# KiloHertzian/Open-Headstage

Hardware: AMD Instinct MI355X
Metric: Msamples/s stereo 48 kHz (4×512-tap HRIR conv + 10-band EQ); % HBM3E peak (higher is better)
Workload: dtype f32

## Files before the change

open_headstage_amd/csrc/eq_kernels.hip:

```cpp
#include "../../include/ohs_hip.h"
#include "kernels.h"
#include "eq_ring2_body.hpp"
#include "eq_ring64_body.hpp"
#include "eq_quad_ring_body.hpp"
#include "tuning.h"
#ifdef OHS_EXPERIMENTS
#include "experiments/eq_ring_v1.hpp"
#endif

#include <atomic>
#include <cstdlib>

namespace ohs {


template <int SHR, bool GATED>
__device__ __forceinline__ void eq_chunk(long long t0, long long n, int j,
                                         float b0, float b1, float b2, float a1, float a2,
                                         float &s1, float &s2, float &prev, float &c)
{
#pragma unroll
    for (int k = 0; k < 16; ++k) {
        float yv = prev;
        if constexpr (SHR != 0) yv = dpp_mov<0x110 + SHR>(prev, prev);
        const float x = dpp_mov<kRowShr1>(c, prev);
        c = dpp_mov<kRowShl1>(yv, c);
        const float out = s1 + b0 * x;
        const float n1 = (s2 + b1 * x) - a1 * out;
        const float n2 = b2 * x - a2 * out;
        if constexpr (GATED) {
            const long long u = t0 + k - j;
            const bool upd = u >= 0 && u < n;
            s1 = upd ? n1 : s1;
            s2 = upd ? n2 : s2;
            prev = upd ? out : x;
        } else {
            s1 = n1; s2 = n2; prev = out;
        }
    }
}

#include "eq_group_asm.inc"
#define EQ_CLOBBERS "v100", "v102", "v104", "v106", "v108", "v109", "v110", "v111", "v112", "v113", "v114", "memory"
template <int SHR>
__device__ __forceinline__ void eq_group_fast(float b0, v2f b12, v2f a12, float &s1, float &s2, float &o, float &c,
                                              float *sp, const float *lp, const float (&x)[8], float (&nx)[8])
{
#define EQ_GROUP_OUTS [s1] "+v"(s1), [s2] "+v"(s2), [o] "+v"(o), [c] "+v"(c), [n0] "=&v"(nx[0]), [n1] "=&v"(nx[1]), \
                      [n2] "=&v"(nx[2]), [n3] "=&v"(nx[3]), [n4] "=&v"(nx[4]), [n5] "=&v"(nx[5]), [n6] "=&v"(nx[6]),   \
                      [n7] "=&v"(nx[7])
#define EQ_GROUP_INS [b0] "v"(b0), [b12] "v"(b12), [a12] "v"(a12), [sp] "v"(sp), [lp] "v"(lp), [x0] "v"(x[0]),          \
                     [x1] "v"(x[1]), [x2] "v"(x[2]), [x3] "v"(x[3]), [x4] "v"(x[4]), [x5] "v"(x[5]), [x6] "v"(x[6]),   \
                     [x7] "v"(x[7])
    if constexpr (SHR != 0) {
        asm volatile(EQ_GROUP_BODY_SHR : EQ_GROUP_OUTS : EQ_GROUP_INS, [shr] "n"(SHR) : EQ_CLOBBERS);
    } else {
        asm volatile(EQ_GROUP_BODY_NOSHR : EQ_GROUP_OUTS : EQ_GROUP_INS : EQ_CLOBBERS);
    }
#undef EQ_GROUP_OUTS
#undef EQ_GROUP_INS
}


template <int SHR>
__global__ __launch_bounds__(64) void k_eq_pass(const float *in, float *out,
                                                long long stream_stride, long long ch_stride,
                                                long long n, int n_chains, const EqPassTable tab,
                                                float *__restrict__ state, int fp_mode)
{
    ohs_set_fp_mode(fp_mode);
    constexpr int NB = 16 - SHR;
    constexpr int G = 8;
    const int lane = threadIdx.x;
    const int j = lane & 15;
    const long long chain = (long long)blockIdx.x * 4 + (lane >> 4);
    const bool live = chain < n_chains;
    const long long wave_base = (long long)blockIdx.x * 4;
    const long long live_rows = n_chains - wave_base < 4 ? n_chains - wave_base : 4;
    const long long cc = live ? chain : wave_base + (lane >> 4) % live_rows;
    const float *src = in + (cc >> 1) * stream_stride + (cc & 1) * ch_stride;
    float *dst = out + (cc >> 1) * stream_stride + (cc & 1) * ch_stride;

    const float b0 = tab.b0[j], b1 = tab.b1[j], b2 = tab.b2[j], a1 = tab.a1[j], a2 = tab.a2[j];
    const int slot = tab.slot[j];
    float s1 = state[(cc * kEqStateSlots + slot) * 2 + 0];
    float s2 = state[(cc * kEqStateSlots + slot) * 2 + 1];
    float prev = 0.0f, c = 0.0f;

    const long long n_chunks = (n - 1 + NB) / 16 + 1;
    const long long n_groups = (n_chunks + G - 1) / G;
    const long long g_fast_end = n / (16 * G) - 1;

    float cur[G], nxt[G];
#pragma unroll
    for (int e = 0; e < G; ++e) {
        const long long xi = (long long)e * 16 + j;
        cur[e] = (xi < n) ? src[xi] : 0.0f;
    }
    long long g = 0;
    while (g < n_groups) {
        if (g >= 1 && g < g_fast_end) {
            for (; g < g_fast_end; ++g) {
                const float *lp = src + (g + 1) * (16 * G) + j;
                float *sp = dst + g * (16 * G) - 16 - NB + j;
                float xs[8];
#pragma unroll
                for (int e = 0; e < G; ++e) { xs[e] = cur[e]; asm volatile("" : "+v"(xs[e])); }
                eq_group_fast<SHR>(b0, (v2f){b1, b2}, (v2f){a1, a2}, s1, s2, prev, c, sp, lp, xs, nxt);
                eq_wait_loads<8>(nxt);
#pragma unroll
                for (int e = 0; e < G; ++e) cur[e] = nxt[e];
            }
            asm volatile("s_waitcnt vmcnt(0)" ::: "memory");
            continue;
        }
#pragma unroll
        for (int e = 0; e < G; ++e) {
            const long long xi = ((g + 1) * G + e) * 16 + j;
            nxt[e] = (xi < n) ? src[xi] : 0.0f;
        }
#pragma unroll
        for (int e = 0; e < G; ++e) {
            const long long q = g * G + e;
            if (q < n_chunks) {
                const long long t0 = q * 16;
                const long long yi = t0 - 16 - NB + j;
                if (yi >= 0 && yi < n) dst[yi] = c;
                c = cur[e];
                if (t0 >= 16 && t0 + 16 <= n)
                    eq_chunk<SHR, false>(t0, n, j, b0, b1, b2, a1, a2, s1, s2, prev, c);
                else
                    eq_chunk<SHR, true>(t0, n, j, b0, b1, b2, a1, a2, s1, s2, prev, c);
            }
        }
#pragma unroll
        for (int e = 0; e < G; ++e) cur[e] = nxt[e];
        ++g;
    }
    {
        const long long yi = n_chunks * 16 - 16 - NB + j;
        if (yi >= 0 && yi < n) dst[yi] = c;
    }
    if (live && j < NB) {
        state[(cc * kEqStateSlots + slot) * 2 + 0] = s1;
        state[(cc * kEqStateSlots + slot) * 2 + 1] = s2;
    }
}

#ifdef OHS_EXPERIMENTS
#include "experiments/eq_ring_v1_kernel.inc"
#endif

#if defined(OHS_EXPERIMENTS) && defined(OHS_EQ_STAMPS)
#include "experiments/eq_stamps.inc"
#else
#define OHS_EQ_STAMP_BEGIN()
#define OHS_EQ_STAMP_END(wave_id)
#endif
__device__ __forceinline__ bool eq_ring_enter(int xcd_lo, int xcd_n, int prio, int fp_mode, long long &wave_id)
{
    unsigned bid = blockIdx.x;
    if (xcd_n != 8) {
        const unsigned x = (bid & 7u) - (unsigned)xcd_lo;
        if (x >= (unsigned)xcd_n) return false;
        bid = (bid >> 3) * (unsigned)xcd_n + x;
    }
    ohs_set_fp_mode(fp_mode);
    if (prio) __builtin_amdgcn_s_setprio(3);
    wave_id = __builtin_amdgcn_readfirstlane((int)(bid * (blockDim.x >> 6) + (threadIdx.x >> 6)));
    return true;
}

__global__ __launch_bounds__(1024) __attribute__((amdgpu_num_vgpr(16))) void k_eq_ring(const float *in, float *out, long long stream_stride,
                                                 long long ch_stride, long long n, int n_chains, int nb,
                                                 const EqPassTable tab, float *__restrict__ state, int prio, int fp_mode,
                                                 int xcd_lo, int xcd_n, unsigned long long *stamps, int wave_ring)
{
    unsigned bid = blockIdx.x;
    if (xcd_n != 8) {
        const unsigned x = (bid & 7u) - (unsigned)xcd_lo;
        if (x >= (unsigned)xcd_n) return;
        bid = (bid >> 3) * (unsigned)xcd_n + x;
    }
    ohs_set_fp_mode(fp_mode);
    if (prio) __builtin_amdgcn_s_setprio(3);
    const long long wave_id = __builtin_amdgcn_readfirstlane((int)(bid * (blockDim.x >> 6) + (threadIdx.x >> 6)));
    OHS_EQ_STAMP_BEGIN();
    const bool stamp = stamps != nullptr && wave_id == 0;
    unsigned long long srt0 = 0, sck0 = 0;
    if (stamp) { srt0 = __builtin_amdgcn_s_memrealtime(); sck0 = __builtin_amdgcn_s_memtime(); }
    const int ring_form = __builtin_amdgcn_readfirstlane(wave_ring);
#ifdef OHS_EXPERIMENTS
    if (ring_form == 3) eq_quad_ring_wave<kQuadLoopFill>(in, out, stream_stride, ch_stride, n, n_chains, nb, tab, state, wave_id);
    else if (ring_form == 4) eq_quad_ring_wave<kQuadLoopLone>(in, out, stream_stride, ch_stride, n, n_chains, nb, tab, state, wave_id);
    else if (ring_form == 5) eq_quad_ring_wave<kQuadLoopCluster>(in, out, stream_stride, ch_stride, n, n_chains, nb, tab, state, wave_id);
    else
#endif
    if (ring_form == 2) eq_quad_ring_wave(in, out, stream_stride, ch_stride, n, n_chains, nb, tab, state, wave_id);
    else if (ring_form) eq_ring64_wave(in, out, stream_stride, ch_stride, n, n_chains, nb, tab, state, wave_id);
    else eq_ring2_wave(in, out, stream_stride, ch_stride, n, n_chains, nb, tab, state, wave_id);
    if (stamp) {
        const unsigned long long srt1 = __builtin_amdgcn_s_memrealtime(), sck1 = __builtin_amdgcn_s_memtime();
        if ((threadIdx.x & 63) == 0) { stamps[0] = srt0; stamps[1] = srt1; stamps[2] = sck0; stamps[3] = sck1; }
    }
    OHS_EQ_STAMP_END(wave_id);
}

__global__ __launch_bounds__(1024) __attribute__((amdgpu_num_vgpr(16))) void k_eq_ring_streams(const float *in, float *out, long long stream_stride,
                                                 long long ch_stride, long long n, int n_chains,
                                                 const EqStreamTable *__restrict__ stabs, float *__restrict__ state, int prio,
                                                 int fp_mode, int xcd_lo, int xcd_n, int wave_ring)
{
    long long wave_id;
    if (!eq_ring_enter(xcd_lo, xcd_n, prio, fp_mode, wave_id)) return;
    EqPassTable unused;
    if (__builtin_amdgcn_readfirstlane(wave_ring)) eq_ring64_wave_t<true>(in, out, stream_stride, ch_stride, n, n_chains, 0, unused, stabs, state, wave_id);
    else eq_ring2_wave_t<true>(in, out, stream_stride, ch_stride, n, n_chains, 0, unused, stabs, state, wave_id);
}

__global__ __launch_bounds__(1024) void k_eq_ring_sched(const float *in, float *out, long long stream_stride, long long ch_stride,
                                                        long long n, int n_chains, int nb, const EqPassTable tab,
                                                        float *__restrict__ state, int prio, int fp_mode, int xcd_lo, int xcd_n,
                                                        unsigned long long *stamps, const EqRingSched sch)
{
    unsigned bid = blockIdx.x;
    if (xcd_n != 8) {
        const unsigned x = (bid & 7u) - (unsigned)xcd_lo;
        if (x >= (unsigned)xcd_n) return;
        bid = (bid >> 3) * (unsigned)xcd_n + x;
    }
    ohs_set_fp_mode(fp_mode);
    if (prio) __builtin_amdgcn_s_setprio(3);
    const long long wave_id = __builtin_amdgcn_readfirstlane((int)(bid * (blockDim.x >> 6) + (threadIdx.x >> 6)));
    const bool stamp = stamps != nullptr && wave_id == 0;
    unsigned long long srt0 = 0, sck0 = 0;
    if (stamp) { srt0 = __builtin_amdgcn_s_memrealtime(); sck0 = __builtin_amdgcn_s_memtime(); }
    eq_ring64_wave_t<false, true>(in, out, stream_stride, ch_stride, n, n_chains, nb, tab, nullptr, state, wave_id, &sch);
    if (stamp) {
        const unsigned long long srt1 = __builtin_amdgcn_s_memrealtime(), sck1 = __builtin_amdgcn_s_memtime();
        if ((threadIdx.x & 63) == 0) { stamps[0] = srt0; stamps[1] = srt1; stamps[2] = sck0; stamps[3] = sck1; }
    }
}

static int eq_device_cus()
{
    static std::atomic<int> cus_cached{0};
    int cus = cus_cached.load(std::memory_order_relaxed);
    if (cus == 0) {
        int dev = 0;
        if (hipGetDevice(&dev) != hipSuccess ||
            hipDeviceGetAttribute(&cus, hipDeviceAttributeMultiprocessorCount, dev) != hipSuccess || cus <= 0)
            cus = 256;
        cus_cached.store(cus, std::memory_order_relaxed);
    }
    return cus;
}

static EqPlan eq_plan_for(bool one_table, long long stream_stride, long long ch_stride, long long n, int n_chains, int n_bands,
                          bool exact_specials, int xcd_lo, int xcd_n)
{
    return eq_plan(one_table, eq_ring2_addressable(stream_stride, ch_stride, n), n, n_chains, n_bands, exact_specials, xcd_lo, xcd_n,
                   eq_device_cus(), tuning());
}

bool eq_pass_takes_wave_ring(long long stream_stride, long long ch_stride, long long n, int n_chains, int n_bands, bool exact_specials)
{
    return eq_plan_for(true, stream_stride, ch_stride, n, n_chains, n_bands, exact_specials, 0, 8).form == OHS_EQ_FORM_WAVE_RING;
}

template <typename... P, typename... A>
static hipError_t eq_dispatch(void (*kernel)(P...), const EqPlan &p, hipStream_t st, hipEvent_t ev_start, hipEvent_t ev_stop, A... args)
{
    if (!p.valid) return hipErrorInvalidValue;
    const bool launch = p.form != OHS_EQ_FORM_NONE;
    const dim3 grid(p.grid), block(64 * p.wg_waves);
    if (launch && p.form != OHS_EQ_FORM_CONVEYOR && !p.ring_v1 && (ev_start || ev_stop)) {
        hipExtLaunchKernelGGL(kernel, grid, block, p.lds, st, ev_start, ev_stop, 0, static_cast<P>(args)...);
        return hipGetLastError();
    }
    if (ev_start) { hipError_t e = hipEventRecord(ev_start, st); if (e != hipSuccess) return e; }
    if (launch) {
        hipLaunchKernelGGL(kernel, grid, block, p.lds, st, static_cast<P>(args)...);
        hipError_t e = hipGetLastError();
        if (e != hipSuccess) return e;
    }
    return ev_stop ? hipEventRecord(ev_stop, st) : hipSuccess;
}

static bool eq_sched_in_bounds(const EqRingSched &sch, long long n)
{
    return sch.lane_tabs && sch.seg_tab && (n & 511) == 0 && sch.seg_len >= 512 && (sch.seg_len & 511) == 0 && (sch.off0 & 511) == 0 &&
           sch.off0 >= 0 && sch.off0 < sch.seg_len && sch.seg0 >= 0 && sch.seg0 < sch.n_segs;
}

hipError_t launch_eq_ring_sched(const float *in, float *out, long long stream_stride, long long ch_stride, long long n, int n_chains,
                                const EqPassTable &tab, int n_bands, float *state, const EqRingSched &sch, hipStream_t st,
                                int fp_mode, int xcd_lo, int xcd_n, hipEvent_t ev_start, hipEvent_t ev_stop, unsigned long long *stamps)
{
    const EqPlan p = eq_plan_for(true, stream_stride, ch_stride, n, n_chains, n_bands, false, xcd_lo, xcd_n);
    if (p.form != OHS_EQ_FORM_WAVE_RING || !eq_sched_in_bounds(sch, n)) return hipErrorInvalidValue;
    return eq_dispatch(k_eq_ring_sched, p, st, ev_start, ev_stop, in, out, stream_stride, ch_stride, n, n_chains, n_bands, tab, state,
                       p.prio, fp_mode, xcd_lo, xcd_n, stamps, sch);
}

__global__ __launch_bounds__(1024) void k_eq_ring_sched_streams(const float *in, float *out, long long stream_stride,
                                                                long long ch_stride, long long n, int n_chains,
                                                                const EqStreamTable *__restrict__ stabs, float *__restrict__ state,
                                                                int prio, int fp_mode, int xcd_lo, int xcd_n, const EqRingSched sch,
                                                                long long idx_stride)
{
    long long wave_id;
    if (!eq_ring_enter(xcd_lo, xcd_n, prio, fp_mode, wave_id)) return;
    EqPassTable unused;
    eq_ring64_wave_t<true, true>(in, out, stream_stride, ch_stride, n, n_chains, 0, unused, stabs, state, wave_id, &sch, idx_stride);
}

hipError_t launch_eq_ring_sched_streams(const float *in, float *out, long long stream_stride, long long ch_stride, long long n,
                                        int n_chains, const EqStreamTable *d_tabs, float *state, const EqRingSched &sch,
                                        long long idx_stride, hipStream_t st, int fp_mode, int xcd_lo, int xcd_n,
                                        hipEvent_t ev_start, hipEvent_t ev_stop)
{
    const EqPlan p = eq_plan_for(true, stream_stride, ch_stride, n, n_chains, 1, false, xcd_lo, xcd_n);
    if (p.form != OHS_EQ_FORM_WAVE_RING || !d_tabs || !eq_sched_in_bounds(sch, n) || (idx_stride != 0 && idx_stride < sch.n_segs))
        return hipErrorInvalidValue;
    return eq_dispatch(k_eq_ring_sched_streams, p, st, ev_start, ev_stop, in, out, stream_stride, ch_stride, n, n_chains, d_tabs, state,
                       p.prio, fp_mode, xcd_lo, xcd_n, sch, idx_stride);
}

__global__ __launch_bounds__(256) void k_eq_gather_tables(unsigned *__restrict__ dst, const unsigned *__restrict__ tabs,
                                                          const unsigned *__restrict__ idx, long long idx_stride, int n_streams,
                                                          int n_tables, int passes)
{
    constexpr int W = (int)(sizeof(EqStreamTable) / 4);
    const long long i = (long long)blockIdx.x * blockDim.x + threadIdx.x;
    if (i >= (long long)passes * n_streams * W) return;
    const int w = (int)(i % W);
    const long long ps = i / W;
    const int s = (int)(ps % n_streams), pk = (int)(ps / n_streams);
    const unsigned t = idx[(long long)s * idx_stride];
    if (t >= (unsigned)n_tables) return;
    dst[i] = tabs[((long long)pk * n_tables + t) * W + w];
}
hipError_t launch_eq_gather_tables(EqStreamTable *dst, const EqStreamTable *tabs, const unsigned *idx, long long idx_stride,
                                   int n_streams, int n_tables, int passes, hipStream_t st)
{
    static_assert(sizeof(EqStreamTable) % 4 == 0, "EqStreamTable is copied word by word");
    if (!dst || !tabs || !idx || idx_stride < 0 || n_streams <= 0 || n_tables <= 0 || passes <= 0) return hipErrorInvalidValue;
    const long long words = (long long)passes * n_streams * (long long)(sizeof(EqStreamTable) / 4);
    hipLaunchKernelGGL(k_eq_gather_tables, dim3((unsigned)((words + 255) / 256)), dim3(256), 0, st, reinterpret_cast<unsigned *>(dst),
                       reinterpret_cast<const unsigned *>(tabs), idx, idx_stride, n_streams, n_tables, passes);
    return hipGetLastError();
}

bool eq_ring_addressable(long long stream_stride, long long ch_stride, long long n)
{
    return eq_ring2_addressable(stream_stride, ch_stride, n);
}

hipError_t launch_eq_ring_streams(const float *in, float *out, long long stream_stride, long long ch_stride, long long n,
                                  int n_chains, const EqStreamTable *d_tabs, float *state, hipStream_t st, int fp_mode,
                                  int xcd_lo, int xcd_n, hipEvent_t ev_start, hipEvent_t ev_stop, int *form)
{
    EqPlan p = eq_plan_for(false, stream_stride, ch_stride, n, n_chains, 0, false, xcd_lo, xcd_n);
    if (p.form != OHS_EQ_FORM_NONE && !d_tabs) p = EqPlan();
    if (form) *form = p.form;
    return eq_dispatch(k_eq_ring_streams, p, st, ev_start, ev_stop, in, out, stream_stride, ch_stride, n, n_chains, d_tabs, state,
                       p.prio, fp_mode, xcd_lo, xcd_n, p.body);
}

hipError_t launch_eq_pass(const float *in, float *out, long long stream_stride, long long ch_stride,
                          long long n, int n_chains, const EqPassTable &tab, int n_bands, float *state,
                          hipStream_t st, bool exact_specials, int fp_mode, int xcd_lo, int xcd_n,
                          hipEvent_t ev_start, hipEvent_t ev_stop, unsigned long long *stamps, int *form)
{
    const EqPlan p = eq_plan_for(true, stream_stride, ch_stride, n, n_chains, n_bands, exact_specials, xcd_lo, xcd_n);
    if (form) *form = p.form;
    if (p.form == OHS_EQ_FORM_CONVEYOR) {
#define OHS_EQ_CASE(NBV)                                                                                              \
    case NBV:                                                                                                         \
        return eq_dispatch(k_eq_pass<16 - NBV>, p, st, ev_start, ev_stop, in, out, stream_stride, ch_stride, n, n_chains, tab, state, \
                           fp_mode);
        switch (n_bands) {
            OHS_EQ_CASE(1) OHS_EQ_CASE(2) OHS_EQ_CASE(3) OHS_EQ_CASE(4) OHS_EQ_CASE(5) OHS_EQ_CASE(6)
            OHS_EQ_CASE(7) OHS_EQ_CASE(8) OHS_EQ_CASE(9) OHS_EQ_CASE(10) OHS_EQ_CASE(11) OHS_EQ_CASE(12)
            OHS_EQ_CASE(13) OHS_EQ_CASE(14) OHS_EQ_CASE(15) OHS_EQ_CASE(16)
        }
#undef OHS_EQ_CASE
        return hipErrorInvalidValue;
    }
#ifdef OHS_EXPERIMENTS
    if (p.ring_v1)
        return eq_dispatch(k_eq_ring_v1, p, st, ev_start, ev_stop, in, out, stream_stride, ch_stride, n, n_chains, n_bands, tab, state,
                           fp_mode);
#endif
    return eq_dispatch(k_eq_ring, p, st, ev_start, ev_stop, in, out, stream_stride, ch_stride, n, n_chains, n_bands, tab, state, p.prio,
                       fp_mode, xcd_lo, xcd_n, stamps, p.body);
}

__global__ void k_eq_freq_response(const float *__restrict__ coeffs, const int *__restrict__ en, int nb,
                                   float fs, const float *__restrict__ freqs, int n, float *__restrict__ out)
{
    const int i = blockIdx.x * blockDim.x + threadIdx.x;
    if (i >= n) return;
    const float pi = 3.14159265358979323846264338327950288f;
    float rr = 1.0f, ri = 0.0f;
    for (int b = 0; b < nb; ++b) {
        if (!en[b]) continue;
        const float b0 = coeffs[5 * b], b1 = coeffs[5 * b + 1], b2 = coeffs[5 * b + 2];
        const float a1 = coeffs[5 * b + 3], a2 = coeffs[5 * b + 4];
        const float omega = 2.0f * pi * freqs[i] / fs;
        const float zr = 1.0f * cosf(-omega), zi = 1.0f * sinf(-omega);
        const float ns = zr * zr + zi * zi;
        const float ir = zr / ns, ii = -zi / ns;
        const float i2r = ir * ir - ii * ii, i2i = ir * ii + ii * ir;
        const float nr = (b0 + b1 * ir) + b2 * i2r, ni = b1 * ii + b2 * i2i;
        const float dr = (1.0f + a1 * ir) + a2 * i2r, di = a1 * ii + a2 * i2i;
        const float dn = dr * dr + di * di;
        const float qr = (nr * dr + ni * di) / dn, qi = (ni * dr - nr * di) / dn;
        const float tr = rr * qr - ri * qi, ti = rr * qi + ri * qr;
        rr = tr; ri = ti;
    }
    out[i] = hypotf(rr, ri);
}

hipError_t launch_eq_freq_response(const float *d_coeffs, const int *d_en, int nb, float fs,
                                   const float *d_freqs, int n, float *d_out, hipStream_t st)
{
    if (n <= 0) return hipSuccess;
    hipLaunchKernelGGL(k_eq_freq_response, dim3((n + 63) / 64), dim3(64), 0, st, d_coeffs, d_en, nb, fs,
                       d_freqs, n, d_out);
    return hipGetLastError();
}

}
```

open_headstage_amd/csrc/eq_plan.h:

```cpp
#pragma once

#include "../../include/ohs_hip.h"
#include "tuning.h"

namespace ohs {

inline unsigned xcd_grid(unsigned workgroups, int xcd_n)
{
    return xcd_n == 8 ? workgroups : ((workgroups + (unsigned)xcd_n - 1) / (unsigned)xcd_n) * 8u;
}

struct EqPlan {
    bool valid = false;
    int form = OHS_EQ_FORM_NONE;
    int body = 0;
    bool ring_v1 = false;
    int wg_waves = 1;
    unsigned grid = 0;
    int prio = 0;
    int lds = 0;
};

inline EqPlan eq_plan(bool one_table, bool addressable, long long n, int n_chains, int n_bands, bool exact_specials, int xcd_lo,
                      int xcd_n, int cus, const Tuning &tn)
{
    EqPlan p;
    if (n <= 0 || n_chains <= 0) { p.valid = true; return p; }
    if (one_table ? (n_bands < 1 || n_bands > 16) : ((n_chains & 1) || !addressable)) return p;
    bool ring_v1 = false;
#ifdef OHS_EXPERIMENTS
    ring_v1 = one_table && tn.eq_ring_v1 != 0;
#endif
    const int blocks = (n_chains + 3) / 4;
    if (one_table && (n_bands > 12 || tn.eq_conveyor || exact_specials || !(ring_v1 || addressable))) {
        p.valid = true;
        p.form = OHS_EQ_FORM_CONVEYOR;
        p.grid = (unsigned)blocks;
        return p;
    }
    const bool wave_ring = !ring_v1 && (tn.eq_form == 2 || tn.eq_form == 3 || (tn.eq_form == 0 && n_chains <= 2 * cus && n >= 8192));
    const int waves = wave_ring ? n_chains : blocks;
    const int wg_override = (ring_v1 && tn.eq_wg_waves > 4) ? 0 : tn.eq_wg_waves;
    p.wg_waves = wg_override ? wg_override : (wave_ring ? 1 : (blocks >= cus ? 4 : 1));
    const unsigned workgroups = (unsigned)((waves + p.wg_waves - 1) / p.wg_waves);
    p.ring_v1 = ring_v1;
    if (ring_v1) {
        p.grid = workgroups;
    } else {
        if (xcd_n < 1 || xcd_n > 8 || xcd_lo < 0 || xcd_lo + xcd_n > 8) return EqPlan();
        p.grid = xcd_grid(workgroups, xcd_n);
        p.prio = tn.eq_no_prio ? 0 : 1;
        p.lds = tn.eq_lds;
#ifdef OHS_EXPERIMENTS
        p.body = !wave_ring ? 0 : (!one_table || tn.eq_form == 2) ? 1 : tn.eq_quad_fill ? 3 : tn.eq_quad_lone_port ? 4 :
                 tn.eq_quad_cluster_port ? 5 : 2;
#else
        p.body = !wave_ring ? 0 : (!one_table || tn.eq_form == 2) ? 1 : 2;
#endif
    }
    p.valid = true;
    p.form = wave_ring ? OHS_EQ_FORM_WAVE_RING : OHS_EQ_FORM_ROW_RING;
    return p;
}

}
```

open_headstage_amd/csrc/eq_quad_ring_body.hpp:

```cpp
#pragma once
#include "kernels.h"
#include "eq_ring64_body.hpp"
#include "eq_quad_ring_asm.inc"
#include "eq_quad_ring_cl_asm.inc"
#include "eq_quad_ring_mg_asm.inc"
#include <type_traits>

namespace ohs {

constexpr int kQuadGroup = 16;
constexpr int kQuadK = EQ_QUAD_RING_K;
constexpr int kQp0003 = 0xC0, kQp0033 = 0xF0, kQp0012 = 0x90, kQp0101 = 0x44;

struct QuadRegs { float Z0, Z1, Zp, G, P; };
enum { kQuadLoopMerged, kQuadLoopCluster, kQuadLoopLone, kQuadLoopFill };

template <int CTRL>
__device__ __forceinline__ float quad_dpp(float src)
{
    return __int_as_float(__builtin_amdgcn_update_dpp(0, __float_as_int(src), CTRL, 0xf, 0xf, true));
}

template <int LOOP = kQuadLoopMerged>
__device__ __forceinline__ void eq_quad_ring_wave(const float *in, float *out, long long stream_stride, long long ch_stride,
                                                  long long n, int n_chains, int nb, const EqPassTable &tab,
                                                  float *__restrict__ state, long long chain)
{
    constexpr int G = kQuadGroup, K = kQuadK;
    static_assert(K == 8, "the operand list below names x0 .. x7");
    static_assert(EQ_QUAD_RING_CL_HOLD == 1 && EQ_QUAD_RING_MG_HOLD == 1, "the clobber lists below name one holding register, v20");
    static_assert(EQ_QUAD_RING_MG_PAIRS == 0, "the operand list below is that of one load and one store per group");
    if (chain >= n_chains) return;
    const int lane = threadIdx.x & 63, q = lane >> 2, role = lane & 3;
    const int n32 = (int)n;
    const bool band = q < nb, conv = q >= 12;
    const int j = band ? q : 0;
    const float C1 = role < 2 ? 1.0f : !band ? 0.0f : role == 2 ? tab.a2[j] : tab.a1[j];
    const float C2 = !band ? (role < 2 ? 0.0f : 1.0f) : role == 0 ? tab.b2[j] : role == 1 ? tab.b1[j] : role == 2 ? tab.b0[j] : 1.0f;
    const long long base = (chain >> 1) * stream_stride + (chain & 1) * ch_stride;
    const float *src0 = in + base;
    float *dst0 = out + base;
    float *state0 = state + chain * (kEqStateSlots * 2);
    const bool st_band = band && role >= 2;
    const unsigned state_off = (unsigned)(tab.slot[j] * 2 + (role == 2 ? 1 : 0)) * 4u;
    const float s_init = st_band ? ring2_ld(state0, state_off) : 0.0f;
    float s_save = s_init;
    const int t_in = 4 * q + 2;
    const int xs = (role == 0 ? 71 : role == 1 ? 69 : role == 2 ? 62 : 60) - 4 * q;
    const int ss = (role == 0 ? -1 : -3) - 4 * q;
    const bool st_lane = conv && (role == 0 || role == 3), inj_lane = conv && role >= 2;
    auto load_x = [&](int g) -> float {
        const int i = g * G + xs;
        return (conv && (unsigned)i < (unsigned)n32) ? ring2_ld(src0, (unsigned)i * 4u) : 0.0f;
    };
    QuadRegs r = {0.0f, 0.0f, 0.0f, 0.0f, 0.0f};
    float xcur = load_x(-1), xnext = load_x(0);

    const int g_hi = (n32 + 1) / G;
    const int iters = g_hi - 5 >= K ? (g_hi - 5) / K : 0;
    const int g1 = iters ? g_hi : -1, g0 = iters ? g_hi - iters * K : -1;
    float x2 = 0.0f, x3 = 0.0f, x4 = 0.0f, x5 = 0.0f, x6 = 0.0f, x7 = 0.0f;
    if (iters) {
        x2 = load_x(g0 + 2); x3 = load_x(g0 + 3); x4 = load_x(g0 + 4);
        x5 = load_x(g0 + 5); x6 = load_x(g0 + 6); x7 = load_x(g0 + 7);
    }

    enum { kPlain, kStore, kInjectB, kInjectA };
    auto group_cpp = [&](int g, auto with_state) {
        constexpr bool STATE = decltype(with_state)::value;
        const float xnext2 = load_x(g + 2);
        auto step = [&](auto kind, float &zc, const float zo, int s) {
            const int stp = g * G + s;
            zc = quad_dpp<kWaveRor1>(r.Zp) + r.G;
            r.Zp = quad_dpp<kQp0003>(zo) * C2;
            if constexpr (kind() == kStore) {
                const int yi = stp + ss;
                if (st_lane && (unsigned)yi < (unsigned)n32) ring2_st(dst0, (unsigned)yi * 4u, zc);
            } else if constexpr (kind() == kInjectB) {
                const float xb = quad_dpp<kQp0101>(xcur);
                r.Zp = inj_lane ? xb : r.Zp;
            } else if constexpr (kind() == kInjectA) {
                r.Zp = inj_lane ? xnext : r.Zp;
            }
            r.P = quad_dpp<kQp0033>(zc) * C1;
            r.G = quad_dpp<kQp0012>(zc) - r.P;
            if constexpr (STATE) {
                r.G = (st_band && stp == t_in) ? s_init : r.G;
                s_save = (st_band && stp == n32 + t_in) ? r.G : s_save;
            }
        };
        using Plain = std::integral_constant<int, kPlain>;
        auto plain_pairs = [&](int s0, int s1) {
#pragma unroll 1
            for (int s = s0; s < s1; s += 2) {
                step(Plain{}, r.Z1, r.Z0, s);
                step(Plain{}, r.Z0, r.Z1, s + 1);
            }
        };
        plain_pairs(1, 6);
        step(Plain{}, r.Z1, r.Z0, 7);
        step(std::integral_constant<int, kStore>{}, r.Z0, r.Z1, 8);
        step(std::integral_constant<int, kInjectB>{}, r.Z1, r.Z0, 9);
        step(Plain{}, r.Z0, r.Z1, 10);
        plain_pairs(11, 14);
        step(std::integral_constant<int, kStore>{}, r.Z1, r.Z0, 15);
        step(std::integral_constant<int, kInjectA>{}, r.Z0, r.Z1, 16);
        xcur = xnext;
        xnext = xnext2;
    };

    const int g_total = (n32 + 62 + G - 1) / G;
    int g = -1;
    const int head_end = iters ? g0 : g_total;
#pragma unroll 1
    for (; g < head_end && (g < 3 || !iters); ++g) group_cpp(g, std::true_type{});
#pragma unroll 1
    for (; g < head_end; ++g) group_cpp(g, std::false_type{});
    if (iters) {
        const unsigned bytes = (unsigned)n32 * 4u;
        const ring64_rsrc_t rin = ring64_rsrc(src0, bytes), rout = ring64_rsrc(dst0, bytes);
        constexpr bool kMerged = LOOP == kQuadLoopMerged;
        const int ms = (role == 0 ? -1 : role == 1 ? -8 : role == 2 ? -10 : -3) - 4 * q;
        unsigned voff_st = kMerged ? (conv ? (unsigned)(G * (g0 - 1) + 15 + ms) * 4u - 28u : 0xFFFFF000u)
                                   : (st_lane ? (unsigned)(G * (g0 - 1) + 8 + ss) * 4u : 0xFFFFF000u);
        unsigned voff_ld = conv ? (unsigned)(G * g0 + xs) * 4u : 0xFFFFF000u;
        const unsigned inc_ld = conv ? 4u * G * K : 0u, inc_st = (kMerged ? conv : st_lane) ? 4u * G * K : 0u;
        unsigned cnt = 0u - (unsigned)__builtin_amdgcn_readfirstlane(iters);
#ifdef OHS_EXPERIMENTS
        if constexpr (LOOP == kQuadLoopFill) {
            unsigned fill = 0u;
            asm volatile(
                "s_nop 4\n"
                EQ_QUAD_RING_LOOP_FILL
                : [Z0] "+{v2}"(r.Z0), [Z1] "+{v3}"(r.Z1), [Zp] "+{v4}"(r.Zp), [Gr] "+{v5}"(r.G), [P] "+{v6}"(r.P),
                  [vs] "+{v0}"(voff_st), [vl] "+{v1}"(voff_ld), [x0] "+{v11}"(xcur), [x1] "+{v12}"(xnext), [x2] "+{v13}"(x2),
                  [x3] "+{v14}"(x3), [x4] "+{v15}"(x4), [x5] "+{v16}"(x5), [x6] "+{v17}"(x6), [x7] "+{v18}"(x7),
                  [F] "+{v19}"(fill), [cnt] "+s"(cnt)
                : [C1] "{v7}"(C1), [C2] "{v8}"(C2), [incl] "{v9}"(inc_ld), [incs] "{v10}"(inc_st), [rin] "s"(rin), [rout] "s"(rout)
                : "memory", "scc", "vcc");
        } else if constexpr (LOOP == kQuadLoopLone) {
            asm volatile(
                "s_nop 4\n"
                EQ_QUAD_RING_LOOP
                : [Z0] "+{v2}"(r.Z0), [Z1] "+{v3}"(r.Z1), [Zp] "+{v4}"(r.Zp), [Gr] "+{v5}"(r.G), [P] "+{v6}"(r.P),
                  [vs] "+{v0}"(voff_st), [vl] "+{v1}"(voff_ld), [x0] "+{v11}"(xcur), [x1] "+{v12}"(xnext), [x2] "+{v13}"(x2),
                  [x3] "+{v14}"(x3), [x4] "+{v15}"(x4), [x5] "+{v16}"(x5), [x6] "+{v17}"(x6), [x7] "+{v18}"(x7), [cnt] "+s"(cnt)
                : [C1] "{v7}"(C1), [C2] "{v8}"(C2), [incl] "{v9}"(inc_ld), [incs] "{v10}"(inc_st), [rin] "s"(rin), [rout] "s"(rout)
                : "memory", "scc", "vcc");
        } else if constexpr (LOOP == kQuadLoopCluster) {
            asm volatile(
                "s_nop 4\n"
                EQ_QUAD_RING_CL_LOOP
                : [Z0] "+{v2}"(r.Z0), [Z1] "+{v3}"(r.Z1), [Zp] "+{v4}"(r.Zp), [Gr] "+{v5}"(r.G), [P] "+{v6}"(r.P),
                  [vs] "+{v0}"(voff_st), [vl] "+{v1}"(voff_ld), [x0] "+{v11}"(xcur), [x1] "+{v12}"(xnext), [x2] "+{v13}"(x2),
                  [x3] "+{v14}"(x3), [x4] "+{v15}"(x4), [x5] "+{v16}"(x5), [x6] "+{v17}"(x6), [x7] "+{v18}"(x7), [cnt] "+s"(cnt)
                : [C1] "{v7}"(C1), [C2] "{v8}"(C2), [incl] "{v9}"(inc_ld), [incs] "{v10}"(inc_st), [rin] "s"(rin), [rout] "s"(rout)
                : "memory", "scc", "vcc", "v20");
        } else
#endif
        {
            static_assert(LOOP == kQuadLoopMerged, "the product library has the merged loop only");
            const unsigned long long mk = 0x9999999999999999ull;
            asm volatile(
                "s_nop 4\n"
                EQ_QUAD_RING_MG_LOOP
                : [Z0] "+{v2}"(r.Z0), [Z1] "+{v3}"(r.Z1), [Zp] "+{v4}"(r.Zp), [Gr] "+{v5}"(r.G), [P] "+{v6}"(r.P),
                  [vs] "+{v0}"(voff_st), [vl] "+{v1}"(voff_ld), [x0] "+{v11}"(xcur), [x1] "+{v12}"(xnext), [x2] "+{v13}"(x2),
                  [x3] "+{v14}"(x3), [x4] "+{v15}"(x4), [x5] "+{v16}"(x5), [x6] "+{v17}"(x6), [x7] "+{v18}"(x7), [cnt] "+s"(cnt)
                : [C1] "{v7}"(C1), [C2] "{v8}"(C2), [incl] "{v9}"(inc_ld), [incs] "{v10}"(inc_st), [rin] "s"(rin), [rout] "s"(rout),
                  [mk] "s"(mk)
                : "memory", "scc", "vcc", "v20");
        }
        g = g1;
#pragma unroll 1
        for (; g < g_total; ++g) group_cpp(g, std::true_type{});
    }
    if (st_band) ring2_st(state0, state_off, s_save);
}

}
```

open_headstage_amd/csrc/tuning.cpp:

```cpp
#include "tuning.h"

#include <algorithm>
#include <cstdio>
#include <cstdlib>
#include <mutex>

namespace ohs {

namespace {
Tuning g_tuning;

#ifdef OHS_EXPERIMENTS
bool parse_ints(const std::string &v, int *out, int n)
{
    const char *p = v.c_str();
    for (int i = 0; i < n; ++i) {
        char *end = nullptr;
        const long x = strtol(p, &end, 10);
        if (end == p) return false;
        out[i] = (int)x;
        p = (*end == ',') ? end + 1 : end;
    }
    return true;
}

const struct { const char *env, *key; } kEnvKeys[] = {
    {"OHS_P1_TARGET_WAVES", "p1_target_waves"}, {"OHS_P1_ROUNDS", "p1_rounds"}, {"OHS_P1_OWN_TAILS", "p1_own_tails"},
    {"OHS_P1_STAGGER", "p1_stagger"}, {"OHS_P1_PRIO", "p1_prio"}, {"OHS_P1_WEIGHTS", "p1_weights"},
    {"OHS_P1_LAZY_STATE", "p1_lazy_state"}, {"OHS_P1_XCD", "p1_xcd"}, {"OHS_EQ_XCD", "eq_xcd"},
    {"OHS_EQ_CONVEYOR", "eq_conveyor"}, {"OHS_EQ_RING_V1", "eq_ring_v1"}, {"OHS_EQ_NO_PRIO", "eq_no_prio"}, {"OHS_EQ_FORM", "eq_form"},
    {"OHS_EQ_QUAD_FILL", "eq_quad_fill"}, {"OHS_EQ_QUAD_LONE_PORT", "eq_quad_lone_port"},
    {"OHS_EQ_QUAD_CLUSTER_PORT", "eq_quad_cluster_port"},
    {"OHS_EQ_WG_WAVES", "eq_wg_waves"}, {"OHS_EQ_LDS", "eq_lds"}, {"OHS_NO_OVERLAP", "no_overlap"},
    {"OHS_FORCE_OVERLAP", "force_overlap"}, {"OHS_XCD_SPLIT", "xcd_split"}, {"OHS_OVERLAP_CUTS", "overlap_cuts"},
    {"OHS_CONV_CU_MASK", "conv_cu_mask"}, {"OHS_MAC_NO_XCD", "mac_no_xcd"}, {"OHS_HOST_PIPE_TRACE", "host_pipe_trace"},
    {"OHS_HOST_PIPE_FLAT_PRIORITIES", "host_pipe_flat_priorities"}, {"OHS_RT_MAX_RESIDENT", "rt_max_resident"},
    {"OHS_RT_IDLE_POLLS", "rt_idle_polls"}, {"OHS_RT_POLL_SLEEP", "rt_poll_sleep"},
    {"OHS_NODE_SHARED_DEVICE", "node_shared_device_rehearsal"},
};
std::once_flag g_env_once;
void load_env()
{
    for (const auto &e : kEnvKeys)
        if (const char *v = getenv(e.env))
            if (!tuning_set(e.key, v)) fprintf(stderr, "[ohs experiments] %s=%s ignored\n", e.env, v);
}
#endif
}

const Tuning &tuning()
{
#ifdef OHS_EXPERIMENTS
    std::call_once(g_env_once, load_env);
#endif
    return g_tuning;
}

Tuning &tuning_rt()
{
#ifdef OHS_EXPERIMENTS
    std::call_once(g_env_once, load_env);
#endif
    return g_tuning;
}

#ifdef OHS_EXPERIMENTS
bool tuning_set(const std::string &key, const std::string &value)
{
    Tuning &t = g_tuning;
    int v[4] = {0, 0, 0, 0};
    auto one = [&](int *dst) { if (!parse_ints(value, v, 1)) return false; *dst = v[0]; return true; };
    if (key == "p1_target_waves") { t.p1_target_waves = atoll(value.c_str()); return true; }
    if (key == "p1_rounds") return one(&t.p1_rounds) && (t.p1_rounds = (t.p1_rounds >= 1 && t.p1_rounds <= 4) ? t.p1_rounds : 1);
    if (key == "p1_own_tails") return one(&t.p1_own_tails);
    if (key == "p1_stagger") return one(&t.p1_stagger);
    if (key == "p1_prio") return one(&t.p1_prio);
    if (key == "p1_lazy_state") return one(&t.p1_lazy_state);
    if (key == "p1_weights") {
        if (!parse_ints(value, v, 4)) return false;
        for (int i = 0; i < 4; ++i) if (v[i] <= 0 || v[i] >= 100000) return false;
        for (int i = 0; i < 4; ++i) t.p1_weights[i] = v[i];
        return true;
    }
    if (key == "p1_xcd" || key == "eq_xcd") {
        int *lo = key == "p1_xcd" ? &t.p1_xcd_lo : &t.eq_xcd_lo, *n = key == "p1_xcd" ? &t.p1_xcd_n : &t.eq_xcd_n;
        if (value.empty() || value == "off") { *lo = 0; *n = 0; return true; }
        if (!parse_ints(value, v, 2) || v[1] < 1 || v[0] < 0 || v[0] + v[1] > 8) return false;
        *lo = v[0]; *n = v[1];
        return true;
    }
    if (key == "eq_conveyor") return one(&t.eq_conveyor);
    if (key == "eq_ring_v1") return one(&t.eq_ring_v1);
    if (key == "eq_no_prio") return one(&t.eq_no_prio);
    if (key == "eq_form") return one(&t.eq_form);
    if (key == "eq_quad_fill") return one(&t.eq_quad_fill);
    if (key == "eq_quad_lone_port") return one(&t.eq_quad_lone_port);
    if (key == "eq_quad_cluster_port") return one(&t.eq_quad_cluster_port);
    if (key == "eq_wg_waves") {
        if (!one(&t.eq_wg_waves)) return false;
        const int w = t.eq_wg_waves;
        if (!(w == 0 || w == 1 || w == 2 || w == 4 || w == 8 || w == 16)) { t.eq_wg_waves = 0; return false; }
        return true;
    }
    if (key == "eq_lds") { if (!one(&t.eq_lds)) return false; if (t.eq_lds < 0 || t.eq_lds > 65536) t.eq_lds = 0; return true; }
    if (key == "no_overlap") return one(&t.no_overlap);
    if (key == "force_overlap") return one(&t.force_overlap);
    if (key == "xcd_split") { if (!one(&t.xcd_split)) return false; if (t.xcd_split < 0 || t.xcd_split > 7) t.xcd_split = 0; return true; }
    if (key == "overlap_cuts") {
        std::vector<double> c = {0.0};
        const char *p = value.c_str();
        while (*p && c.size() < 16) {
            char *end = nullptr;
            const double x = strtod(p, &end);
            if (end == p) break;
            if (x > c.back() && x < 1.0) c.push_back(x);
            p = (*end == ',') ? end + 1 : end;
        }
        c.push_back(1.0);
        if (c.size() < 3) return false;
        t.overlap_cuts = c;
        return true;
    }
    if (key == "conv_cu_mask") {
        std::vector<unsigned> m;
        const char *p = value.c_str();
        while (*p) {
            char *end = nullptr;
            const unsigned long x = strtoul(p, &end, 16);
            if (end == p) break;
            m.push_back((unsigned)x);
            p = (*end == ',') ? end + 1 : end;
        }
        t.conv_cu_mask = m;
        return true;
    }
    if (key == "mac_no_xcd") return one(&t.mac_no_xcd);
    if (key == "lb_skip") return one(&t.lb_skip);
    if (key == "xb_min_p") return one(&t.xb_min_p);
    if (key == "xb_min_blocks") return one(&t.xb_min_blocks);
    if (key == "xb_min_streams_p2") return one(&t.xb_min_streams_p2);
    if (key == "xb_stagger") { if (!one(&t.xb_stagger)) return false; t.xb_stagger = std::max(0, std::min(t.xb_stagger, 64)); return true; }
    if (key == "xb_run") return one(&t.xb_run);
    if (key == "xb_skip") return one(&t.xb_skip);
    if (key == "lb_seg_windows") { if (!one(&t.lb_seg_windows)) return false; if (t.lb_seg_windows < 64) t.lb_seg_windows = 64; return true; }
    if (key == "lb_min_p") { if (!one(&t.lb_min_p)) return false; if (t.lb_min_p < 2) t.lb_min_p = 2; return true; }
    if (key == "host_pipe_trace") return one(&t.host_pipe_trace);
    if (key == "host_pipe_flat_priorities") return one(&t.host_pipe_flat_priorities);
    if (key == "node_shared_device_rehearsal") return one(&t.node_shared_device_rehearsal);
    if (key == "node_inject_table_failure_slot") return one(&t.node_inject_table_failure_slot);
    if (key == "rt_max_resident") { int v = 0; if (!one(&v)) return false; rt_max_resident_store(v); return true; }
    if (key == "rt_idle_polls") { rt_idle_polls_store(strtoull(value.c_str(), nullptr, 10)); return true; }
    if (key == "rt_poll_sleep") { if (!one(v)) return false; t.rt_poll_sleep = (unsigned)v[0]; return true; }
    return false;
}
#endif

}
```

open_headstage_amd/csrc/tuning.h:

```cpp
#pragma once
#include "experiments.h"

#include <string>
#include <vector>

namespace ohs {

struct Tuning {
    long long p1_target_waves = 0;
    int p1_rounds = 1;
    int p1_own_tails = 1;
    int p1_stagger = 0;
    int p1_prio = 0;
    int p1_weights[4] = {1425, 1128, 825, 622};
    int p1_lazy_state = 1;
    int p1_xcd_lo = 0, p1_xcd_n = 0;
    int eq_xcd_lo = 0, eq_xcd_n = 0;
    int eq_conveyor = 0;
    int eq_ring_v1 = 0;
    int eq_no_prio = 0;
    int eq_form = 0;
    int eq_quad_fill = 0;
    int eq_quad_lone_port = 0;
    int eq_quad_cluster_port = 0;
    int eq_wg_waves = 0;
    int eq_lds = 0;
    int no_overlap = 0, force_overlap = 0;
    int xcd_split = 0;
    std::vector<double> overlap_cuts = {0.0, 0.25, 0.5, 0.75, 0.92, 0.98, 1.0};
    std::vector<unsigned> conv_cu_mask;
    int mac_no_xcd = 0;
    int lb_min_p = 2;
    int lb_seg_windows = 131072;
    int xb_min_p = 2;
    int xb_min_blocks = 128;
    int xb_min_streams_p2 = 32;
    int xb_stagger = 1;
    int xb_skip = 0;
    int xb_run = 0;
    int lb_skip = 0;
    int host_pipe_trace = 0, host_pipe_flat_priorities = 0;
    int node_shared_device_rehearsal = 0;
    int node_inject_table_failure_slot = 0;
    int rt_max_resident = -1;
    unsigned long long rt_idle_polls = 3000000ull;
    unsigned rt_poll_sleep = 0;
};

const Tuning &tuning();
Tuning &tuning_rt();
inline int rt_max_resident_load() { return __atomic_load_n(&tuning().rt_max_resident, __ATOMIC_RELAXED); }
inline unsigned long long rt_idle_polls_load() { return __atomic_load_n(&tuning().rt_idle_polls, __ATOMIC_RELAXED); }
inline void rt_max_resident_store(int v) { __atomic_store_n(&tuning_rt().rt_max_resident, v, __ATOMIC_RELAXED); }
inline void rt_idle_polls_store(unsigned long long v) { __atomic_store_n(&tuning_rt().rt_idle_polls, v, __ATOMIC_RELAXED); }
#ifdef OHS_EXPERIMENTS
bool tuning_set(const std::string &key, const std::string &value);
#endif

}
```

Baseline: 27920.

## Prefetch quad-ring EQ head groups four ahead with buffer loads and stores

The default (streaming) quad-ring EQ path now issues input loads for the head and tail groups four groups ahead, using rotating registers and raw buffer loads whose out-of-range offsets return zero. Stores use buffer stores with an out-of-bounds offset for masked lanes, and the state and coefficient loads are hoisted and issued unconditionally. The aim is to hide global load latency in the serial edge loops instead of waiting on each group's load. The old waiting behaviour is kept as an experiment-only variant. This adds code size, register pressure and more complex loop-boundary logic.

```diff
diff --git a/open_headstage_amd/csrc/eq_kernels.hip b/open_headstage_amd/csrc/eq_kernels.hip
--- a/open_headstage_amd/csrc/eq_kernels.hip
+++ b/open_headstage_amd/csrc/eq_kernels.hip
@@ -194,6 +194,7 @@
     if (ring_form == 3) eq_quad_ring_wave<kQuadLoopFill>(in, out, stream_stride, ch_stride, n, n_chains, nb, tab, state, wave_id);
     else if (ring_form == 4) eq_quad_ring_wave<kQuadLoopLone>(in, out, stream_stride, ch_stride, n, n_chains, nb, tab, state, wave_id);
     else if (ring_form == 5) eq_quad_ring_wave<kQuadLoopCluster>(in, out, stream_stride, ch_stride, n, n_chains, nb, tab, state, wave_id);
+    else if (ring_form == 6) eq_quad_ring_wave<kQuadLoopMerged, kQuadEdgesWaiting>(in, out, stream_stride, ch_stride, n, n_chains, nb, tab, state, wave_id);
     else
 #endif
     if (ring_form == 2) eq_quad_ring_wave(in, out, stream_stride, ch_stride, n, n_chains, nb, tab, state, wave_id);
diff --git a/open_headstage_amd/csrc/eq_plan.h b/open_headstage_amd/csrc/eq_plan.h
--- a/open_headstage_amd/csrc/eq_plan.h
+++ b/open_headstage_amd/csrc/eq_plan.h
@@ -53,7 +53,7 @@
         p.lds = tn.eq_lds;
 #ifdef OHS_EXPERIMENTS
         p.body = !wave_ring ? 0 : (!one_table || tn.eq_form == 2) ? 1 : tn.eq_quad_fill ? 3 : tn.eq_quad_lone_port ? 4 :
-                 tn.eq_quad_cluster_port ? 5 : 2;
+                 tn.eq_quad_cluster_port ? 5 : tn.eq_quad_waiting_edges ? 6 : 2;
 #else
         p.body = !wave_ring ? 0 : (!one_table || tn.eq_form == 2) ? 1 : 2;
 #endif
diff --git a/open_headstage_amd/csrc/eq_quad_ring_body.hpp b/open_headstage_amd/csrc/eq_quad_ring_body.hpp
--- a/open_headstage_amd/csrc/eq_quad_ring_body.hpp
+++ b/open_headstage_amd/csrc/eq_quad_ring_body.hpp
@@ -14,6 +14,8 @@
 
 struct QuadRegs { float Z0, Z1, Zp, G, P; };
 enum { kQuadLoopMerged, kQuadLoopCluster, kQuadLoopLone, kQuadLoopFill };
+enum { kQuadEdgesStreaming, kQuadEdgesWaiting };
+constexpr unsigned kQuadNoLane = 0xFFFFF000u;
 
 template <int CTRL>
 __device__ __forceinline__ float quad_dpp(float src)
@@ -21,30 +23,38 @@
     return __int_as_float(__builtin_amdgcn_update_dpp(0, __float_as_int(src), CTRL, 0xf, 0xf, true));
 }
 
-template <int LOOP = kQuadLoopMerged>
+template <int LOOP = kQuadLoopMerged, int EDGES = kQuadEdgesStreaming>
 __device__ __forceinline__ void eq_quad_ring_wave(const float *in, float *out, long long stream_stride, long long ch_stride,
                                                   long long n, int n_chains, int nb, const EqPassTable &tab,
                                                   float *__restrict__ state, long long chain)
 {
     constexpr int G = kQuadGroup, K = kQuadK;
+    constexpr bool kWaiting = EDGES == kQuadEdgesWaiting;
     static_assert(K == 8, "the operand list below names x0 .. x7");
     static_assert(EQ_QUAD_RING_CL_HOLD == 1 && EQ_QUAD_RING_MG_HOLD == 1, "the clobber lists below name one holding register, v20");
     static_assert(EQ_QUAD_RING_MG_PAIRS == 0, "the operand list below is that of one load and one store per group");
+#ifndef OHS_EXPERIMENTS
+    static_assert(!kWaiting, "the product library has the streaming edges only");
+#endif
     if (chain >= n_chains) return;
     const int lane = threadIdx.x & 63, q = lane >> 2, role = lane & 3;
     const int n32 = (int)n;
     const bool band = q < nb, conv = q >= 12;
     const int j = band ? q : 0;
-    const float C1 = role < 2 ? 1.0f : !band ? 0.0f : role == 2 ? tab.a2[j] : tab.a1[j];
-    const float C2 = !band ? (role < 2 ? 0.0f : 1.0f) : role == 0 ? tab.b2[j] : role == 1 ? tab.b1[j] : role == 2 ? tab.b0[j] : 1.0f;
+    float C1, C2;
+    if constexpr (kWaiting) {
+        C1 = role < 2 ? 1.0f : !band ? 0.0f : role == 2 ? tab.a2[j] : tab.a1[j];
+        C2 = !band ? (role < 2 ? 0.0f : 1.0f) : role == 0 ? tab.b2[j] : role == 1 ? tab.b1[j] : role == 2 ? tab.b0[j] : 1.0f;
+    } else {
+        const float ta = (role == 2 ? tab.a2 : tab.a1)[j], tb = (role == 0 ? tab.b2 : role == 1 ? tab.b1 : tab.b0)[j];
+        C1 = role < 2 ? 1.0f : !band ? 0.0f : ta;
+        C2 = !band ? (role < 2 ? 0.0f : 1.0f) : role == 3 ? 1.0f : tb;
+    }
     const long long base = (chain >> 1) * stream_stride + (chain & 1) * ch_stride;
     const float *src0 = in + base;
     float *dst0 = out + base;
     float *state0 = state + chain * (kEqStateSlots * 2);
     const bool st_band = band && role >= 2;
-    const unsigned state_off = (unsigned)(tab.slot[j] * 2 + (role == 2 ? 1 : 0)) * 4u;
-    const float s_init = st_band ? ring2_ld(state0, state_off) : 0.0f;
-    float s_save = s_init;
     const int t_in = 4 * q + 2;
     const int xs = (role == 0 ? 71 : role == 1 ? 69 : role == 2 ? 62 : 60) - 4 * q;
     const int ss = (role == 0 ? -1 : -3) - 4 * q;
@@ -53,41 +63,82 @@
         const int i = g * G + xs;
         return (conv && (unsigned)i < (unsigned)n32) ? ring2_ld(src0, (unsigned)i * 4u) : 0.0f;
     };
+    const unsigned n_bytes = (unsigned)n32 * 4u;
+    const __amdgpu_buffer_rsrc_t bin = __builtin_amdgcn_make_buffer_rsrc(const_cast<float *>(src0), 0, (int)n_bytes, 0x00020000),
+                                 bout = __builtin_amdgcn_make_buffer_rsrc(dst0, 0, (int)n_bytes, 0x00020000);
+    auto request_x = [&](int g, bool wanted) -> float {
+        const unsigned off = (conv && wanted) ? (unsigned)(g * G + xs) * 4u : kQuadNoLane;
+        return __uint_as_float(__builtin_amdgcn_raw_buffer_load_b32(bin, off, 0, 0));
+    };
     QuadRegs r = {0.0f, 0.0f, 0.0f, 0.0f, 0.0f};
-    float xcur = load_x(-1), xnext = load_x(0);
 
     const int g_hi = (n32 + 1) / G;
     const int iters = g_hi - 5 >= K ? (g_hi - 5) / K : 0;
     const int g1 = iters ? g_hi : -1, g0 = iters ? g_hi - iters * K : -1;
+    const int g_total = (n32 + 62 + G - 1) / G;
+    const int g_nl = (n32 + G - 1) / G - 2;
+    const int head_end = iters ? g0 : kWaiting ? g_total : g_nl;
+    const int lim = head_end + 1, p0 = (-(head_end + 1)) & 3;
+    float R0 = 0.0f, R1 = 0.0f, R2 = 0.0f, R3 = 0.0f;
+    float xcur = 0.0f, xnext = 0.0f;
     float x2 = 0.0f, x3 = 0.0f, x4 = 0.0f, x5 = 0.0f, x6 = 0.0f, x7 = 0.0f;
-    if (iters) {
-        x2 = load_x(g0 + 2); x3 = load_x(g0 + 3); x4 = load_x(g0 + 4);
-        x5 = load_x(g0 + 5); x6 = load_x(g0 + 6); x7 = load_x(g0 + 7);
-    }
+    unsigned state_off;
+    float s_init;
+    if constexpr (kWaiting) {
+        state_off = (unsigned)(tab.slot[j] * 2 + (role == 2 ? 1 : 0)) * 4u;
+        s_init = st_band ? ring2_ld(state0, state_off) : 0.0f;
+        xcur = load_x(-1); xnext = load_x(0);
+        if (iters) {
+            x2 = load_x(g0 + 2); x3 = load_x(g0 + 3); x4 = load_x(g0 + 4);
+            x5 = load_x(g0 + 5); x6 = load_x(g0 + 6); x7 = load_x(g0 + 7);
+        }
+    } else {
+        const int slot = tab.slot[j];
+        const int gp0 = -1 + ((0 - p0) & 3), gp1 = -1 + ((1 - p0) & 3), gp2 = -1 + ((2 - p0) & 3), gp3 = -1 + ((3 - p0) & 3);
+        R0 = request_x(gp0, gp0 <= lim); R1 = request_x(gp1, gp1 <= lim);
+        R2 = request_x(gp2, gp2 <= lim); R3 = request_x(gp3, gp3 <= lim);
+        const unsigned xo = (conv && iters) ? (unsigned)((g0 + 2) * G + xs) * 4u : kQuadNoLane;
+        x2 = __uint_as_float(__builtin_amdgcn_raw_buffer_load_b32(bin, xo, 0, 0));
+        x3 = __uint_as_float(__builtin_amdgcn_raw_buffer_load_b32(bin, xo + 4u * G, 0, 0));
+        x4 = __uint_as_float(__builtin_amdgcn_raw_buffer_load_b32(bin, xo + 8u * G, 0, 0));
+        x5 = __uint_as_float(__builtin_amdgcn_raw_buffer_load_b32(bin, xo + 12u * G, 0, 0));
+        x6 = __uint_as_float(__builtin_amdgcn_raw_buffer_load_b32(bin, xo + 16u * G, 0, 0));
+        x7 = __uint_as_float(__builtin_amdgcn_raw_buffer_load_b32(bin, xo + 20u * G, 0, 0));
+        state_off = (unsigned)(slot * 2 + (role == 2 ? 1 : 0)) * 4u;
+        const float s_word = ring2_ld(state0, state_off);
+        s_init = st_band ? s_word : 0.0f;
+        asm volatile("" : : "v"(s_init));
+    }
+    float s_save = s_init;
 
     enum { kPlain, kStore, kInjectB, kInjectA };
-    auto group_cpp = [&](int g, auto with_state) {
-        constexpr bool STATE = decltype(with_state)::value;
-        const float xnext2 = load_x(g + 2);
+    enum { kStateNone, kStateIn, kStateInOut };
+    using StateNone = std::integral_constant<int, kStateNone>;
+    using StateIn = std::integral_constant<int, kStateIn>;
+    using StateInOut = std::integral_constant<int, kStateInOut>;
+    auto group_steps = [&](int g, auto with_state, float &xb, const float &xa, auto &&reload) {
+        constexpr int STATE = decltype(with_state)::value;
         auto step = [&](auto kind, float &zc, const float zo, int s) {
             const int stp = g * G + s;
             zc = quad_dpp<kWaveRor1>(r.Zp) + r.G;
             r.Zp = quad_dpp<kQp0003>(zo) * C2;
             if constexpr (kind() == kStore) {
                 const int yi = stp + ss;
-                if (st_lane && (unsigned)yi < (unsigned)n32) ring2_st(dst0, (unsigned)yi * 4u, zc);
+                if constexpr (kWaiting) {
+                    if (st_lane && (unsigned)yi < (unsigned)n32) ring2_st(dst0, (unsigned)yi * 4u, zc);
+                } else {
+                    __builtin_amdgcn_raw_buffer_store_b32(__float_as_uint(zc), bout, st_lane ? (unsigned)yi * 4u : kQuadNoLane, 0, 0);
+                }
             } else if constexpr (kind() == kInjectB) {
-                const float xb = quad_dpp<kQp0101>(xcur);
-                r.Zp = inj_lane ? xb : r.Zp;
+                const float xq = quad_dpp<kQp0101>(xb);
+                r.Zp = inj_lane ? xq : r.Zp;
             } else if constexpr (kind() == kInjectA) {
-                r.Zp = inj_lane ? xnext : r.Zp;
+                r.Zp = inj_lane ? xa : r.Zp;
             }
             r.P = quad_dpp<kQp0033>(zc) * C1;
             r.G = quad_dpp<kQp0012>(zc) - r.P;
-            if constexpr (STATE) {
-                r.G = (st_band && stp == t_in) ? s_init : r.G;
-                s_save = (st_band && stp == n32 + t_in) ? r.G : s_save;
-            }
+            if constexpr (STATE != kStateNone) r.G = (st_band && stp == t_in) ? s_init : r.G;
+            if constexpr (STATE == kStateInOut) s_save = (st_band && stp == n32 + t_in) ? r.G : s_save;
         };
         using Plain = std::integral_constant<int, kPlain>;
         auto plain_pairs = [&](int s0, int s1) {
@@ -101,21 +152,53 @@
         step(Plain{}, r.Z1, r.Z0, 7);
         step(std::integral_constant<int, kStore>{}, r.Z0, r.Z1, 8);
         step(std::integral_constant<int, kInjectB>{}, r.Z1, r.Z0, 9);
+        reload(xb);
         step(Plain{}, r.Z0, r.Z1, 10);
         plain_pairs(11, 14);
         step(std::integral_constant<int, kStore>{}, r.Z1, r.Z0, 15);
         step(std::integral_constant<int, kInjectA>{}, r.Z0, r.Z1, 16);
+    };
+    auto group_cpp = [&](int g, auto with_state) {
+        const float xnext2 = load_x(g + 2);
+        group_steps(g, with_state, xcur, xnext, [](float &) {});
         xcur = xnext;
         xnext = xnext2;
     };
-
-    const int g_total = (n32 + 62 + G - 1) / G;
+    auto group_head = [&](int g, auto with_state, float &xb, const float &xa) {
+        group_steps(g, with_state, xb, xa, [&](float &x) { x = request_x(g + 4, g + 4 <= lim); });
+    };
+    auto block_head = [&](int g, auto with_state) {
+        group_head(g, with_state, R0, R1);
+        group_head(g + 1, with_state, R1, R2);
+        group_head(g + 2, with_state, R2, R3);
+        group_head(g + 3, with_state, R3, R0);
+    };
+    auto group_tail = [&](int g) {
+        group_steps(g, StateInOut{}, xcur, xnext, [](float &) {});
+        xcur = xnext;
+        xnext = 0.0f;
+    };
+
     int g = -1;
-    const int head_end = iters ? g0 : g_total;
-#pragma unroll 1
-    for (; g < head_end && (g < 3 || !iters); ++g) group_cpp(g, std::true_type{});
-#pragma unroll 1
-    for (; g < head_end; ++g) group_cpp(g, std::false_type{});
+    if constexpr (kWaiting) {
+#pragma unroll 1
+        for (; g < head_end && (g < 3 || !iters); ++g) group_cpp(g, StateInOut{});
+#pragma unroll 1
+        for (; g < head_end; ++g) group_cpp(g, StateNone{});
+    } else {
+        switch ((head_end + 1) & 3) {
+        case 3: group_head(g, StateIn{}, R1, R2); ++g; [[fallthrough]];
+        case 2: group_head(g, StateIn{}, R2, R3); ++g; [[fallthrough]];
+        case 1: group_head(g, StateIn{}, R3, R0); ++g; [[fallthrough]];
+        default: break;
+        }
+#pragma unroll 1
+        for (; g < head_end && (g < 3 || !iters); g += 4) block_head(g, StateIn{});
+#pragma unroll 1
+        for (; g < head_end; g += 4) block_head(g, StateNone{});
+        xcur = R0;
+        xnext = R1;
+    }
     if (iters) {
         const unsigned bytes = (unsigned)n32 * 4u;
         const ring64_rsrc_t rin = ring64_rsrc(src0, bytes), rout = ring64_rsrc(dst0, bytes);
@@ -172,8 +255,14 @@
                 : "memory", "scc", "vcc", "v20");
         }
         g = g1;
-#pragma unroll 1
-        for (; g < g_total; ++g) group_cpp(g, std::true_type{});
+        if constexpr (kWaiting) {
+#pragma unroll 1
+            for (; g < g_total; ++g) group_cpp(g, StateInOut{});
+        }
+    }
+    if constexpr (!kWaiting) {
+#pragma unroll 1
+        for (; g < g_total; ++g) group_tail(g);
     }
     if (st_band) ring2_st(state0, state_off, s_save);
 }
diff --git a/open_headstage_amd/csrc/tuning.cpp b/open_headstage_amd/csrc/tuning.cpp
--- a/open_headstage_amd/csrc/tuning.cpp
+++ b/open_headstage_amd/csrc/tuning.cpp
@@ -30,7 +30,7 @@
     {"OHS_P1_LAZY_STATE", "p1_lazy_state"}, {"OHS_P1_XCD", "p1_xcd"}, {"OHS_EQ_XCD", "eq_xcd"},
     {"OHS_EQ_CONVEYOR", "eq_conveyor"}, {"OHS_EQ_RING_V1", "eq_ring_v1"}, {"OHS_EQ_NO_PRIO", "eq_no_prio"}, {"OHS_EQ_FORM", "eq_form"},
     {"OHS_EQ_QUAD_FILL", "eq_quad_fill"}, {"OHS_EQ_QUAD_LONE_PORT", "eq_quad_lone_port"},
-    {"OHS_EQ_QUAD_CLUSTER_PORT", "eq_quad_cluster_port"},
+    {"OHS_EQ_QUAD_CLUSTER_PORT", "eq_quad_cluster_port"}, {"OHS_EQ_QUAD_WAITING_EDGES", "eq_quad_waiting_edges"},
     {"OHS_EQ_WG_WAVES", "eq_wg_waves"}, {"OHS_EQ_LDS", "eq_lds"}, {"OHS_NO_OVERLAP", "no_overlap"},
     {"OHS_FORCE_OVERLAP", "force_overlap"}, {"OHS_XCD_SPLIT", "xcd_split"}, {"OHS_OVERLAP_CUTS", "overlap_cuts"},
     {"OHS_CONV_CU_MASK", "conv_cu_mask"}, {"OHS_MAC_NO_XCD", "mac_no_xcd"}, {"OHS_HOST_PIPE_TRACE", "host_pipe_trace"},
@@ -96,6 +96,7 @@
     if (key == "eq_quad_fill") return one(&t.eq_quad_fill);
     if (key == "eq_quad_lone_port") return one(&t.eq_quad_lone_port);
     if (key == "eq_quad_cluster_port") return one(&t.eq_quad_cluster_port);
+    if (key == "eq_quad_waiting_edges") return one(&t.eq_quad_waiting_edges);
     if (key == "eq_wg_waves") {
         if (!one(&t.eq_wg_waves)) return false;
         const int w = t.eq_wg_waves;
diff --git a/open_headstage_amd/csrc/tuning.h b/open_headstage_amd/csrc/tuning.h
--- a/open_headstage_amd/csrc/tuning.h
+++ b/open_headstage_amd/csrc/tuning.h
@@ -23,6 +23,7 @@
     int eq_quad_fill = 0;
     int eq_quad_lone_port = 0;
     int eq_quad_cluster_port = 0;
+    int eq_quad_waiting_edges = 0;
     int eq_wg_waves = 0;
     int eq_lds = 0;
     int no_overlap = 0, force_overlap = 0;
```

Result: no change. 28040 (median of 6 runs) (+0.4%).
